# zovoilis-lab/Flye

Hardware: AMD Instinct MI355X
Metric: Gbp reads overlapped/sec (higher is better)
Workload: dtype u64

## Files before the change

### flye_amd/csrc/fg_ctx.h

```cpp
#pragma once

#include <hip/hip_runtime.h>
#include <cstdint>
#include <cstdio>
#include <cstdlib>
#include <new>
#include <cstring>
#include <string>
#include <vector>
#include <map>
#include <memory>
#include <condition_variable>
#include <functional>
#include <mutex>
#include <thread>
#include <atomic>
#include <algorithm>

#include "../../include/flye_gpu.h"
#include "fg_error.h"

typedef uint64_t u64;
typedef uint32_t u32;
typedef uint16_t u16;
// ... 255 lines not shown

	bool indexBuilt = false;
	float sampleRate = 1.0f;
	u64 nKeys = 0, nEntries = 0, nRep = 0, tableSlots = 0;
	DevBuf<u64> dKeys;
	DevBuf<u64> dKeyOff;
	DevBuf<u64> dEntries;
	DevBuf<u64> dRepKeys;
	DevBuf<u64> dTable;
	bool tableWide = false;
	FgTable table{};
	DevBuf<u32> dIndexedBits;
	DevBuf<u32> dMaybeBits;
	u32 shardWorld = 1, shardRank = 0;

	std::unique_ptr<fg_ctx> lane2;
	std::shared_ptr<void> indexBuild;
	bool gathering = false;
	DevBuf<u64> gKeys, gKeyOff, gEntries, gRepKeys;
	u64 gNKeys = 0, gNEntries = 0, gNRep = 0;
	u32 splitWorld = 0;
	DevBuf<u64> sCounts, sEntries;
	bool scattering = false;
	u32 scatterWorld = 1, scatterRank = 0;

	DevBuf<u32> dQuery;
	u64 hitCapHint = 0;
	const u32* curQuery = nullptr;
	DevBuf<u64> dQKmerOff;
	DevBuf<u64> dProbe;
	DevBuf<u64> dPartK0, dPartV0, dPartK1, dPartV1;
	DevBuf<char> dPartScratch;
	DevBuf<unsigned long long> dPartCount;
	DevBuf<u64> dHitOff;
	DevBuf<u64> dFiltOff;
	DevBuf<i32> dFiltPos;
	DevBuf<u64> dHitKey;
	DevBuf<u32> dHitVal;
	DevBuf<u16> dHitVal16;
	bool hitVal16 = false;
	DevBuf<u32> dHitKey32;
	DevBuf<i32> dScore, dBack;
	DevBuf<int4> dCand;
	DevBuf<u64> dGroupStart;
	DevBuf<u32> dGroupQuery;
	DevBuf<u32> dGroupExt, dGroupFirstCur, dGroupLastCur;
	DevBuf<uint8_t> dGroupExtSorted;
	DevBuf<u32> dTmp32;
	DevBuf<fg_seed_hit> dSeedHits;
	DevBuf<u64> dRecvRun, dRecvIdx;
	DevBuf<u32> dRecvErr;
	DevBuf<u64> dCntA, dCntB, dGroupCnt, dGroupOff, dPrimCnt, dPrimOff, dDpGroups, dDpElems;
	DevBuf<u32> dPrimFlag, dDpSize, dListSmall, dListBig, dListDp, dListFused, dListCnt;
	DevBuf<u32> dCur, dExt;
	DevBuf<char> dPrimOut;
	DevBuf<u64> dPrimNode, dPrimBase, dMatchSize, dMatchOff, dMatches;
	DevBuf<u32> dMatchCnt;
	PinnedBuf<u64> hMatches, hMatchOff;
	PinnedBuf<u32> hMatchCnt;
	DevBuf<char> dSortTasks, dSortBig;
	DevBuf<unsigned long long> dSmallElems;
	DevBuf<unsigned long long> dLazyCnt;
	DevBuf<u32> dSortCnt;
	DevBuf<u32> dTieFree;
	u32 tieFreeQ0 = 0, tieFreeN = 0;
	DevBuf<u32> dSortFree, dSortReason;
	u32 sortReasonN = 0;
	u32 sortRadixSegs = 0;
	DevBuf<int> dEditScratch;
	DevBuf<u32> dEditList;
	DevBuf<char> dEditCnt;
	DevBuf<u64> dEditSlab;
	DevBuf<char> dEditPrims;
	DevBuf<u32> dEditQuery;
	DevBuf<i32> dEditOut;
	DevBuf<char> dRangeSides;
	DevBuf<i32> dRangeLen;
	DevBuf<u64> dRangeOff;
	DevBuf<uint8_t> dRangeTrg, dRangeQry;
	DevBuf<u32> dDecCnt;
	DevBuf<u64> dDecOff;
	DevBuf<uint8_t> dDecOps;
	DevBuf<i32> dDecLens;
	DevBuf<i32> dTrimPre;
	DevBuf<u64> dTrimRowCnt, dTrimRowOff, dTrimScan, dTrimKeys, dTrimIvl, dTrimSeg, dTrimAcc, dTrimAccOff;
	DevBuf<unsigned long long> dTrimPairCnt;
	DevBuf<u32> dTrimVals, dTrimAccCnt, dTrimKept;
	DevBuf<char> dTrimRaw, dTrimOut;
	DevBuf<u32> dRcNodes, dRcVals, dRcU32;
	DevBuf<char> dRcTab, dRcAln;
	DevBuf<u64> dRcOff, dRcKeys, dRcOut;
	DevBuf<i32> dRcOutScore;
	DevBuf<char> dCovRecs, dCovSort;
	DevBuf<u64> dCovIv, dCovKeys, dCovOff;
	DevBuf<i32> dCovI32, dCovVec;
	DevBuf<char> dPolBytes, dPolCand, dPolItems, dPolTasks, dPolRes;
	DevBuf<u64> dPolOff, dPolEdOff;
	DevBuf<long long> dPolScore, dPolCells, dPolEdits;
	DevBuf<char> dBub[36];
	DevBuf<char> dCc[40];
	DevBuf<char> dCig[20];
	DevBuf<char> dDv[28];
	DevBuf<char> dPt[36];
	PinnedBuf<char> hPrim;
	PinnedBuf<u64> hOff;
	PinnedBuf<u64> hScalar;
// ... 2 lines not shown
	~fg_ctx()
	{
		if (evFork) (void)hipEventDestroy(evFork);
		if (evJoin) (void)hipEventDestroy(evJoin);
		if (evJoin3) (void)hipEventDestroy(evJoin3);
		if (evOff) (void)hipEventDestroy(evOff);
		for (auto e : evPiece) if (e) (void)hipEventDestroy(e);
		if (stream2) (void)hipStreamDestroy(stream2);
		if (stream3) (void)hipStreamDestroy(stream3);
		if (stream) (void)hipStreamDestroy(stream);
	}
};

#if defined(__HIPCC__)

__device__ __forceinline__ i32 fg_uni(i32 v) { return __builtin_amdgcn_readfirstlane(v); }
__device__ __forceinline__ u32 fg_uni(u32 v) { return (u32)__builtin_amdgcn_readfirstlane((int)v); }
__device__ __forceinline__ u64 fg_uni(u64 v)
{
	return ((u64)(u32)__builtin_amdgcn_readfirstlane((int)(u32)(v >> 32)) << 32) |
		   (u32)__builtin_amdgcn_readfirstlane((int)(u32)v);
}

#define FG_PK_VALBITS 24
struct PK {
	u64 v;
	PK() = default;
	__host__ __device__ PK(int x) : v((u64)(unsigned)x) {}
	__host__ __device__ explicit PK(u64 x) : v(x) {}
};
__device__ __forceinline__ bool operator<(const PK& a, const PK& b) { return (a.v >> FG_PK_VALBITS) < (b.v >> FG_PK_VALBITS); }
__device__ __forceinline__ bool operator>(const PK& a, const PK& b) { return (a.v >> FG_PK_VALBITS) > (b.v >> FG_PK_VALBITS); }
__device__ __forceinline__ bool operator<=(const PK& a, const PK& b) { return (a.v >> FG_PK_VALBITS) <= (b.v >> FG_PK_VALBITS); }
__device__ __forceinline__ bool operator>=(const PK& a, const PK& b) { return (a.v >> FG_PK_VALBITS) >= (b.v >> FG_PK_VALBITS); }
__device__ __forceinline__ bool operator==(const PK& a, const PK& b) { return a.v == b.v; }
__device__ __forceinline__ bool operator!=(const PK& a, const PK& b) { return a.v != b.v; }

struct NoVal {
	struct Ref {
		__device__ __forceinline__ operator u32() const { return 0u; }
		__device__ __forceinline__ const Ref& operator=(u32) const { return *this; }
	};
	__device__ __forceinline__ Ref operator[](long long) const { return Ref{}; }
	__device__ __forceinline__ NoVal operator+(long long) const { return NoVal{}; }
};

struct K32V16;
template <class KT> struct HitKeyView;
template <> struct HitKeyView<u64> {
	const u64* k; const u32* v; int curBits; u32 firstId;
	__device__ __forceinline__ u32 ext(u64 i) const { return (u32)(k[i] >> 32); }
	__device__ __forceinline__ u32 ext_raw(u64 i) const { return (u32)(k[i] >> 32); }
	__device__ __forceinline__ u32 cur(u64 i) const { return (u32)k[i]; }
	__device__ __forceinline__ u32 val(u64 i) const { return v[i]; }
};
template <> struct HitKeyView<u32> {
	const u32* k; const u32* v; int curBits; u32 firstId;
	__device__ __forceinline__ u32 ext(u64 i) const { return (k[i] >> curBits) + firstId; }
	__device__ __forceinline__ u32 ext_raw(u64 i) const { return k[i] >> curBits; }
	__device__ __forceinline__ u32 cur(u64 i) const { return k[i] & ((1u << curBits) - 1u); }
	__device__ __forceinline__ u32 val(u64 i) const { return v[i]; }
};
template <> struct HitKeyView<K32V16> {
	const u32* k; const u16* v; int curBits; u32 firstId;
	__device__ __forceinline__ u32 ext(u64 i) const { return (k[i] >> curBits) + firstId; }
	__device__ __forceinline__ u32 ext_raw(u64 i) const { return k[i] >> curBits; }
	__device__ __forceinline__ u32 cur(u64 i) const { return k[i] & ((1u << curBits) - 1u); }
	__device__ __forceinline__ u32 val(u64 i) const { return v[i]; }
};
template <> struct HitKeyView<PK> {
	const PK* k; const u32* v; int curBits; u32 firstId;
	__device__ __forceinline__ u32 ext(u64 i) const { return (u32)(k[i].v >> (FG_PK_VALBITS + curBits)) + firstId; }
	__device__ __forceinline__ u32 ext_raw(u64 i) const { return (u32)(k[i].v >> (FG_PK_VALBITS + curBits)); }
	__device__ __forceinline__ u32 cur(u64 i) const { return (u32)(k[i].v >> FG_PK_VALBITS) & ((1u << curBits) - 1u); }
	__device__ __forceinline__ u32 val(u64 i) const { return (u32)k[i].v & ((1u << FG_PK_VALBITS) - 1u); }
};

__device__ __forceinline__ u64 fg_mix(u64 x)
{
	x ^= x >> 33; x *= 0xff51afd7ed558ccdULL; x ^= x >> 33;
	x *= 0xc4ceb9fe1a85ec53ULL; x ^= x >> 33;
	return x;
}

__device__ __forceinline__ u32 fg_base_at(const u64* __restrict__ w, i32 L, bool rc, i32 pos)
{
	const i32 p = rc ? L - 1 - pos : pos;
	const u32 b = (u32)((w[p >> 5] >> ((p & 31) * 2)) & 3);
	return rc ? (~b & 3) : b;
}

__device__ __forceinline__ u64 fg_range_step(const u64* __restrict__ w, i32 L, bool rc, i32 start, i32 len, bool hpc,
											 i32 t0, u32& carry, u32& b, bool& keep)
{
	const int lane = threadIdx.x & 63;
	const i32 t = t0 + lane;
	const bool valid = t < len;
	b = valid ? fg_base_at(w, L, rc, start + t) : 0u;
	u32 prev = __shfl_up(b, 1);
	if (lane == 0) prev = carry;
	keep = valid && (!hpc || prev != b);
	carry = __shfl(b, 63);
	return __builtin_amdgcn_ballot_w64(keep);
}

__device__ __forceinline__ u64 fg_kmer_hash(u64 x)
{
	u64 z = (x += 0x9E3779B97F4A7C15ULL);
	z = (z ^ (z >> 30)) * 0xBF58476D1CE4E5B9ULL;
	z = (z ^ (z >> 27)) * 0x94D049BB133111EBULL;
	return z ^ (z >> 31);
}

__device__ __forceinline__ u64 fg_chunk(const u64* __restrict__ w, i32 q, int k)
{
	const int sh = (q & 31) * 2;
	u64 lo = w[q >> 5] >> sh;
	if (sh + 2 * k > 64) lo |= w[(q >> 5) + 1] << (64 - sh);
	return (k == 32) ? lo : (lo & ((1ULL << (2 * k)) - 1));
}

__device__ __forceinline__ u64 fg_rev2(u64 x, int k)
{
	u64 r = __brevll(x);
	r = ((r >> 1) & 0x5555555555555555ULL) | ((r & 0x5555555555555555ULL) << 1);
	return r >> (64 - 2 * k);
}
// ... 192 lines not shown
```

### flye_amd/csrc/fg_overlap.hip

```cpp
#include "fg_ctx.h"
#include "fg_wavesort.h"
#include "fg_devprim.h"
#include "fg_taskchain.h"
#include <atomic>

#include <algorithm>
#include <cmath>
#include <chrono>
#include <functional>
#include <thread>
#include <type_traits>

#define WG 256
#define FLAG_SELF (1ULL << 63)
#define FLAG_FLIP (1ULL << 62)
#define OFF_MASK ((1ULL << 38) - 1)

namespace {

__device__ __forceinline__ u32 block_exscan(u32 v, u32* sh , u32* total)
{
	const int lane = threadIdx.x & 63, w = threadIdx.x >> 6;
	u32 inc = v;
	for (int o = 1; o < 64; o <<= 1)
// ... 1031 lines not shown
	}
}

__global__ void k_prim_gather(const u64* __restrict__ groupOff, const u32* __restrict__ primCount,
							  const u64* __restrict__ groupStart, const u32* __restrict__ groupExt,
							  const u32* __restrict__ gCur, const u32* __restrict__ gExt, const int4* __restrict__ cand,
							  const i32* __restrict__ len, u32 firstId, int k,
							  const u64* __restrict__ filtOff, const i32* __restrict__ filtPos,
							  const u64* __restrict__ primOff, PrimRec* __restrict__ out,
							  u64* __restrict__ primNode, u64* __restrict__ primBase, u64* __restrict__ matchSize)
{
	__shared__ u32 sh[WG / 64 + 1];
	const u32 q = blockIdx.x;
	const u64 b = groupOff[q], e = groupOff[q + 1];
	u64 obase = primOff[q];
	const i32* fp = filtPos + filtOff[q];
	const i32 nf = (i32)(filtOff[q + 1] - filtOff[q]);
	for (u64 i0 = b; i0 < e; i0 += WG)
	{
		const u64 g = i0 + threadIdx.x;
		const u32 cnt = g < e ? primCount[g] : 0u;
		u32 tot;
		const u32 pos = block_exscan(cnt, sh, &tot);
		if (cnt)
		{
			const u64 g0 = groupStart[g];
			const u32 extId = groupExt[g];
			const i32 extLen = len[(extId - firstId) >> 1];
			for (u32 a = 0; a < cnt; ++a)
			{
				const int4 c4 = cand[g0 + a];
				PrimRec r;
				r.query = q; r.extId = extId;
				r.curBegin = (i32)gCur[g0 + c4.x]; r.extBegin = (i32)gExt[g0 + c4.x];
				r.curEnd = (i32)gCur[g0 + c4.y] + k - 1; r.extEnd = (i32)gExt[g0 + c4.y] + k - 1;
				r.extLen = extLen; r.score = c4.w; r.chainLength = c4.z;
				i32 lo = 0, hi = nf;
				while (lo < hi) { const i32 m = (lo + hi) >> 1; if (fp[m] < r.curBegin) lo = m + 1; else hi = m; }
				const i32 first = lo;
				hi = nf;
				while (lo < hi) { const i32 m = (lo + hi) >> 1; if (fp[m] <= r.curEnd) lo = m + 1; else hi = m; }
				r.filtered = lo - first;
				r.editDistance = -1; r.hpcLenCur = 0; r.hpcLenExt = 0;
				out[obase + pos + a] = r;
				if (primNode)
				{
					primNode[obase + pos + a] = g0 + (u64)c4.y;
					primBase[obase + pos + a] = g0;
					matchSize[obase + pos + a] = (u64)c4.z + 2;
				}
			}
		}
		obase += tot;
	}
}

__global__ void k_chain_matches(const PrimRec* __restrict__ prims, u64 nPrim, const u64* __restrict__ primNode,
								const u64* __restrict__ primBase, const u64* __restrict__ matchOff,
								const u32* __restrict__ gCur, const u32* __restrict__ gExt,
								const i32* __restrict__ gBack, int k, u64* __restrict__ matches,
								u32* __restrict__ matchCnt)
{
	const u64 p = (u64)blockIdx.x * blockDim.x + threadIdx.x;
	if (p >= nPrim) return;
	const PrimRec r = prims[p];
	const u64 base = primBase[p];
	u64* slot = matches + matchOff[p];
	const i32 ub = r.chainLength + 2;
	i32 pos = (i32)(primNode[p] - base);
	i32 kept = 0, lastCur = 0;
	for (i32 step = 0; step < r.chainLength; ++step)
	{
		const i32 cu = (i32)gCur[base + pos];
		if (kept == 0 || lastCur - cu > k)
		{
			slot[ub - 2 - kept] = (u64)(u32)cu | ((u64)gExt[base + pos] << 32);
			lastCur = cu;
			++kept;
		}
		pos = gBack[base + pos];
	}
	slot[ub - 2 - kept] = (u64)(u32)r.curBegin | ((u64)(u32)r.extBegin << 32);
	slot[ub - 1] = (u64)(u32)r.curEnd | ((u64)(u32)r.extEnd << 32);
	matchCnt[p] = (u32)kept + 2;
}

template <class T>
T fetchScalar(fg_ctx* c, const T* dptr)
{
	static_assert(sizeof(T) <= 8, "scalar");
	c->hScalar.reserve(8);
	HIP_CHECK(hipMemcpyAsync(c->hScalar.p, dptr, sizeof(T), hipMemcpyDeviceToHost, c->stream));
	HIP_CHECK(hipStreamSynchronize(c->stream));
	T v;
	memcpy(&v, c->hScalar.p, sizeof(T));
	return v;
}

}

struct SortRadixStats { u64 segments, hits; };

#define SORT_MAX_LEVELS 128
template <class KT>
static bool sortRadixUsable(int recBits)
{
// ... 459 lines not shown
	while ((1ULL << recBits) < 2ULL * c->nReads) ++recBits;
	const bool key32 = curBits + recBits <= 32 && !getenv("FG_FORCE_KEY64");
	c->tieFreeN = 0; c->sortReasonN = 0;
	const bool canPack = recBits + curBits + FG_PK_VALBITS <= 64 && c->maxLen < (1 << FG_PK_VALBITS);
	const bool wantPack = !(getenv("FG_PACKED_KEYS") && atoi(getenv("FG_PACKED_KEYS")) == 0);
	const int keyMode = key32 ? 0 : ((canPack && wantPack) ? 1 : 2);
	const bool val16 = keyMode == 0 && !recv && c->maxLen <= 65536 && !(getenv("FG_VAL16") && atoi(getenv("FG_VAL16")) == 0);
	c->hitVal16 = val16;
	if (keyMode == 0)
	{
		c->dHitKey32.reserve(hitCap + 1); c->dTieFree.reserve(nq + 1);
		if (val16) c->dHitVal16.reserve(hitCap + 2); else c->dHitVal.reserve(hitCap + 1);
		if (recv) recvFill<u32>(c, recv, callQ0, sub0, nq, nHits, curBits, c->dHitKey32.p, c->dHitVal.p);
		else { ScopedK t(c->timer, "k_fill");
		  if (val16)
			  hipLaunchKernelGGL((k_fill<u32, u16>), nq, WG, 0, s, dQuery, c->dLen.p, qLen, dQKmerOff, k, c->firstId, curBits,
								 c->dProbe.p, c->dEntries.p, c->dHitOff.p, c->dFiltOff.p, c->dHitKey32.p, c->dHitVal16.p, c->dFiltPos.p, c->dTieFree.p);
		  else
			  hipLaunchKernelGGL(k_fill<u32>, nq, WG, 0, s, dQuery, c->dLen.p, qLen, dQKmerOff, k, c->firstId, curBits,
								 c->dProbe.p, c->dEntries.p, c->dHitOff.p, c->dFiltOff.p, c->dHitKey32.p, c->dHitVal.p, c->dFiltPos.p, c->dTieFree.p); }
		if (!recv) { c->tieFreeQ0 = callQ0 + sub0; c->tieFreeN = nq; }
		const u32* sortFree = recv ? nullptr : c->dTieFree.p;
		if (sortFree && nHits)
		{
			c->dSortFree.reserve(nq + 1); c->dSortReason.reserve(nq + 1);
			if (sortScreen(c, c->dHitOff.p, nq, c->dHitKey32.p, curBits, recBits, c->dTieFree.p, fgChainMinUnique(p), p->min_overlap,
						   c->dSortFree.p, c->dSortReason.p))
				{ sortFree = c->dSortFree.p; c->sortReasonN = nq; }
		}
		if (val16) sortSegments<u32, u16>(c, c->dHitOff.p, nq, c->dHitKey32.p, c->dHitVal16.p, nHits, curBits, sortFree, recBits);
		else sortSegments<u32>(c, c->dHitOff.p, nq, c->dHitKey32.p, c->dHitVal.p, nHits, curBits, sortFree, recBits);
	}
	else if (keyMode == 1)
	{
		c->dHitKey.reserve(hitCap + 1);
		if (recv) recvFill<PK>(c, recv, callQ0, sub0, nq, nHits, curBits, (PK*)c->dHitKey.p, (u32*)nullptr);
		else { ScopedK t(c->timer, "k_fill");
		  hipLaunchKernelGGL(k_fill<PK>, nq, WG, 0, s, dQuery, c->dLen.p, qLen, dQKmerOff, k, c->firstId, curBits,
							 c->dProbe.p, c->dEntries.p, c->dHitOff.p, c->dFiltOff.p, (PK*)c->dHitKey.p, (u32*)nullptr, c->dFiltPos.p, (u32*)nullptr); }
		sortSegments<PK>(c, c->dHitOff.p, nq, (PK*)c->dHitKey.p, (u32*)nullptr, nHits, curBits);
	}
	else
	{
		c->dHitKey.reserve(hitCap + 1); c->dHitVal.reserve(hitCap + 1);
		if (recv) recvFill<u64>(c, recv, callQ0, sub0, nq, nHits, curBits, c->dHitKey.p, c->dHitVal.p);
		else { ScopedK t(c->timer, "k_fill");
		  hipLaunchKernelGGL(k_fill<u64>, nq, WG, 0, s, dQuery, c->dLen.p, qLen, dQKmerOff, k, c->firstId, 0,
							 c->dProbe.p, c->dEntries.p, c->dHitOff.p, c->dFiltOff.p, c->dHitKey.p, c->dHitVal.p, c->dFiltPos.p, (u32*)nullptr); }
		sortSegments<u64>(c, c->dHitOff.p, nq, c->dHitKey.p, c->dHitVal.p, nHits, curBits);
	}
	const HitKeyView<u32> hk32{c->dHitKey32.p, c->dHitVal.p, curBits, c->firstId};
	const HitKeyView<u64> hk64{c->dHitKey.p, c->dHitVal.p, curBits, c->firstId};
	const HitKeyView<PK> hkp{(const PK*)c->dHitKey.p, nullptr, curBits, c->firstId};
	{ ScopedK t(c->timer, "k_group_count");
	  if (keyMode == 0) hipLaunchKernelGGL(k_group_count<u32>, nq, WG, 0, s, c->dHitOff.p, hk32, c->dGroupCnt.p);
	  else if (keyMode == 1) hipLaunchKernelGGL(k_group_count<PK>, nq, WG, 0, s, c->dHitOff.p, hkp, c->dGroupCnt.p);
	  else hipLaunchKernelGGL(k_group_count<u64>, nq, WG, 0, s, c->dHitOff.p, hk64, c->dGroupCnt.p); }
	{ ScopedK t(c->timer, "k_exscan");
	  hipLaunchKernelGGL(k_exscan, 1, 1024, 0, s, c->dGroupCnt.p, c->dGroupOff.p, nq); }
	const u64 nGroups = fetchScalar(c, c->dGroupOff.p + nq);
	if (nGroups >= 0xFFFFFFFFULL) throw FgError{FG_ERR_ARG, "too many target groups in one chunk"};
	c->dGroupStart.reserve(nGroups + 1); c->dGroupQuery.reserve(nGroups + 1);
	c->dGroupExt.reserve(nGroups + 1); c->dGroupFirstCur.reserve(nGroups + 1); c->dGroupLastCur.reserve(nGroups + 1);
	c->dPrimFlag.reserve(nGroups + 1); c->dDpSize.reserve(nGroups + 1);
	{ ScopedK t(c->timer, "k_group_fill");
	  if (keyMode == 0) hipLaunchKernelGGL(k_group_fill<u32>, nq, WG, 0, s, c->dHitOff.p, hk32, c->dGroupOff.p, c->dGroupStart.p,
										   c->dGroupQuery.p, c->dGroupExt.p, c->dGroupFirstCur.p, c->dGroupLastCur.p);
	  else if (keyMode == 1) hipLaunchKernelGGL(k_group_fill<PK>, nq, WG, 0, s, c->dHitOff.p, hkp, c->dGroupOff.p, c->dGroupStart.p,
												c->dGroupQuery.p, c->dGroupExt.p, c->dGroupFirstCur.p, c->dGroupLastCur.p);
	  else hipLaunchKernelGGL(k_group_fill<u64>, nq, WG, 0, s, c->dHitOff.p, hk64, c->dGroupOff.p, c->dGroupStart.p,
							  c->dGroupQuery.p, c->dGroupExt.p, c->dGroupFirstCur.p, c->dGroupLastCur.p); }
	fgChainStage(c, p, forceLocal, nGroups, nHits, keyMode, curBits);
	c->dSmallElems.reserve(1);
	HIP_CHECK(hipMemsetAsync(c->dSmallElems.p, 0, 8, s));
	{ ScopedK t(c->timer, "k_prim_count");
	  hipLaunchKernelGGL(k_prim_count, nq, WG, 0, s, c->dGroupOff.p, c->dPrimFlag.p, c->dDpSize.p, c->dPrimCnt.p,
						 c->dDpGroups.p, c->dDpElems.p, c->dGroupStart.p, nGroups, nHits, fgChainSmallMax(), c->dSmallElems.p); }
	{ ScopedK t(c->timer, "k_exscan");
	  hipLaunchKernelGGL(k_exscan, 1, 1024, 0, s, c->dPrimCnt.p, c->dPrimOff.p, nq); }
	const u64 nPrim = fetchScalar(c, c->dPrimOff.p + nq);
	c->dPrimOut.reserve((nPrim + 1) * sizeof(PrimRec));
	const bool keepAln = p->keep_alignment;
	if (keepAln) { c->dPrimNode.reserve(nPrim + 1); c->dPrimBase.reserve(nPrim + 1); c->dMatchSize.reserve(nPrim + 1);
				   c->dMatchOff.reserve(nPrim + 2); c->dMatchCnt.reserve(nPrim + 1); }
	{ ScopedK t(c->timer, "k_prim_gather");
	  hipLaunchKernelGGL(k_prim_gather, nq, WG, 0, s, c->dGroupOff.p, c->dPrimFlag.p, c->dGroupStart.p, c->dGroupExt.p,
						 c->dCur.p, c->dExt.p, c->dCand.p, c->dLen.p, c->firstId, k, c->dFiltOff.p, c->dFiltPos.p,
						 c->dPrimOff.p, (PrimRec*)c->dPrimOut.p, keepAln ? c->dPrimNode.p : (u64*)nullptr,
						 keepAln ? c->dPrimBase.p : (u64*)nullptr, keepAln ? c->dMatchSize.p : (u64*)nullptr); }
	if (p->nucl_alignment) fgEditDistances(c, (PrimRec*)c->dPrimOut.p, nPrim, p->use_hpc);
	res->nMatchSlots = 0;
	if (keepAln && nPrim)
	{
		if (nPrim >= 0xFFFFFFFFULL) throw FgError{FG_ERR_ARG, "too many overlaps in one chunk"};
		{ ScopedK t(c->timer, "k_exscan");
		  hipLaunchKernelGGL(k_exscan, 1, 1024, 0, s, c->dMatchSize.p, c->dMatchOff.p, (u32)nPrim); }
		const u64 slots = fetchScalar(c, c->dMatchOff.p + nPrim);
		res->nMatchSlots = slots;
		c->dMatches.reserve(slots + 1);
		{ ScopedK t(c->timer, "k_chain_matches");
		  hipLaunchKernelGGL(k_chain_matches, (unsigned)((nPrim + WG - 1) / WG), WG, 0, s, (const PrimRec*)c->dPrimOut.p, nPrim,
							 c->dPrimNode.p, c->dPrimBase.p, c->dMatchOff.p, c->dCur.p, c->dExt.p, c->dBack.p, k,
							 c->dMatches.p, c->dMatchCnt.p); }
		c->hMatches.reserve(slots + 1); c->hMatchOff.reserve(nPrim + 1); c->hMatchCnt.reserve(nPrim + 1);
		ScopedK t(c->timer, "copy_results_d2h");
		HIP_CHECK(hipMemcpyAsync(c->hMatches.p, c->dMatches.p, slots * 8, hipMemcpyDeviceToHost, s));
		HIP_CHECK(hipMemcpyAsync(c->hMatchOff.p, c->dMatchOff.p, (nPrim + 1) * 8, hipMemcpyDeviceToHost, s));
		HIP_CHECK(hipMemcpyAsync(c->hMatchCnt.p, c->dMatchCnt.p, nPrim * 4, hipMemcpyDeviceToHost, s));
	}
	if ((primBase + nPrim + 1) * sizeof(PrimRec) > c->hPrim.n)
	{
		HIP_CHECK(hipStreamSynchronize(s));
		c->hPrim.reserveKeep((primBase + nPrim + 1) * sizeof(PrimRec), primBase * sizeof(PrimRec));
	}
	c->hOff.reserve(3 * (size_t)(nq + 1) + 1);
	{ ScopedK t(c->timer, "copy_results_d2h");
	  HIP_CHECK(hipMemcpyAsync(c->hOff.p, c->dPrimOff.p, (nq + 1) * 8ULL, hipMemcpyDeviceToHost, s));
	  HIP_CHECK(hipMemcpyAsync(c->hOff.p + (nq + 1), c->dDpGroups.p, nq * 8ULL, hipMemcpyDeviceToHost, s));
	  HIP_CHECK(hipMemcpyAsync(c->hOff.p + 2 * (size_t)(nq + 1), c->dDpElems.p, nq * 8ULL, hipMemcpyDeviceToHost, s));
	  HIP_CHECK(hipMemcpyAsync(c->hOff.p + 3 * (size_t)(nq + 1), c->dSmallElems.p, 8, hipMemcpyDeviceToHost, s));
	  HIP_CHECK(hipEventRecord(c->evOff, s));
	  static const int wantPieces = getenv("FG_D2H_PIECES") ? std::max(1, std::min(FG_D2H_MAX_PIECES, atoi(getenv("FG_D2H_PIECES")))) : 12;
	  const int nPieces = nPrim >= 100000 ? wantPieces : 1;
	  for (int i = 0; i < nPieces; ++i)
	  {
		  const u64 a = nPrim * i / nPieces, b = nPrim * (i + 1) / nPieces;
		  if (b > a)
			  HIP_CHECK(hipMemcpyAsync(c->hPrim.p + (primBase + a) * sizeof(PrimRec), c->dPrimOut.p + a * sizeof(PrimRec),
									   (b - a) * sizeof(PrimRec), hipMemcpyDeviceToHost, s));
		  HIP_CHECK(hipEventRecord(c->evPiece[i], s));
		  c->pieceEnd[i] = primBase + b;
	  }
	  c->nPieces = nPieces; }
	HIP_CHECK(hipEventSynchronize(c->evOff));
	if (keepAln) HIP_CHECK(hipStreamSynchronize(s));
	res->nPrim = nPrim;
	res->dpGroups = 0; res->dpElems = 0;
	res->dpElemsSmall = c->hOff.p[3 * (size_t)(nq + 1)];
	for (u32 i = 0; i < nq; ++i) { res->dpGroups += c->hOff.p[(nq + 1) + i]; res->dpElems += c->hOff.p[2 * (size_t)(nq + 1) + i]; }
}

static void stageBudgets(fg_ctx* c, u64& kmerBudget, u64& hitBudget)
{
	kmerBudget = getenv("FG_KMER_BUDGET") ? strtoull(getenv("FG_KMER_BUDGET"), nullptr, 10) : (1ULL << 30);
	hitBudget = getenv("FG_HIT_BUDGET") ? strtoull(getenv("FG_HIT_BUDGET"), nullptr, 10) : (3ULL << 29);
	if (!getenv("FG_KMER_BUDGET") && !getenv("FG_HIT_BUDGET"))
	{
		size_t freeB = 0, totalB = 0;
		HIP_CHECK(hipMemGetInfo(&freeB, &totalB));
		const u64 held = c->dHitKey.bytes() + c->dHitKey32.bytes() + c->dHitVal.bytes() + c->dHitVal16.bytes() + c->dCur.bytes() + c->dExt.bytes() +
						 c->dScore.bytes() + c->dBack.bytes() + c->dTmp32.bytes() + c->dCand.bytes() + c->dProbe.bytes();
		const u64 avail = (u64)freeB + held;
		const u64 usable = avail > (8ULL << 30) ? (avail - (4ULL << 30)) / 10 * 9 : avail / 2;
		hitBudget = std::min(hitBudget, std::max<u64>(16ULL << 20, usable / 100 * 85 / 80));
		kmerBudget = std::min(kmerBudget, std::max<u64>(16ULL << 20, usable / 100 * 15 / 9));
	}
}

static fg_ctx* laneTwo(fg_ctx* c)
{
	if (!c->lane2)
	{
		std::unique_ptr<fg_ctx> l(new fg_ctx);
		l->device = c->device;
		if (hipStreamCreateWithFlags(&l->stream, hipStreamNonBlocking) != hipSuccess ||
			hipStreamCreateWithFlags(&l->stream2, hipStreamNonBlocking) != hipSuccess ||
			hipStreamCreateWithFlags(&l->stream3, hipStreamNonBlocking) != hipSuccess ||
			hipEventCreateWithFlags(&l->evJoin3, hipEventDisableTiming) != hipSuccess ||
			hipEventCreateWithFlags(&l->evOff, hipEventDisableTiming) != hipSuccess ||
			hipEventCreateWithFlags(&l->evFork, hipEventDisableTiming) != hipSuccess ||
			hipEventCreateWithFlags(&l->evJoin, hipEventDisableTiming) != hipSuccess)
			throw FgError{FG_ERR_HIP, "streams of the second lane"};
		for (auto& e : l->evPiece)
			if (hipEventCreateWithFlags(&e, hipEventDisableTiming) != hipSuccess) throw FgError{FG_ERR_HIP, "events of the second lane"};
		l->timer.stream = l->stream;
		c->lane2 = std::move(l);
	}
	fg_ctx* l = c->lane2.get();
	l->k = c->k; l->nReads = c->nReads; l->firstId = c->firstId; l->maxLen = c->maxLen;
	l->totalKmers = c->totalKmers; l->totalBases = c->totalBases;
	l->hasQ = c->hasQ; l->nQReads = c->nQReads; l->qFirstId = c->qFirstId; l->qMaxLen = c->qMaxLen;
	l->indexBuilt = c->indexBuilt; l->sampleRate = c->sampleRate; l->nKeys = c->nKeys; l->nEntries = c->nEntries; l->nRep = c->nRep;
	l->tableSlots = c->tableSlots; l->tableWide = c->tableWide; l->table = c->table;
	l->timer.enabled = c->timer.enabled;
	l->dWords.alias(c->dWords); l->dWordOff.alias(c->dWordOff); l->dLen.alias(c->dLen); l->dKmerOff.alias(c->dKmerOff);
	l->dQWords.alias(c->dQWords); l->dQWordOff.alias(c->dQWordOff); l->dQLen.alias(c->dQLen);
	l->dKeyOff.alias(c->dKeyOff); l->dEntries.alias(c->dEntries); l->dTable.alias(c->dTable); l->dIndexedBits.alias(c->dIndexedBits); l->dMaybeBits.alias(c->dMaybeBits);
	l->dQuery.alias(c->dQuery); l->dQKmerOff.alias(c->dQKmerOff); l->dProbe.alias(c->dProbe);
	l->dCntA.alias(c->dCntA); l->dCntB.alias(c->dCntB);
	l->dLazyCnt.alias(c->dLazyCnt);
	return l;
}
// ... 475 lines not shown
```

Before: 5.406.

## Flatten group count/fill and primitive scan over hits instead of per-query blocks

Replaces the per-query block launches for group counting, group filling, primitive counting and gathering with flat tile-parallel kernels over all hits, each thread handling 8 consecutive keys. Query boundaries inside a tile are found by binary search and marked in shared memory. The single-block exscan is replaced by a device-wide scan, and per-group primitive positions come from scanning the primitive flags. DP totals are now reduced on the device with atomics instead of being summed on the host from per-query arrays. This removes load imbalance from skewed query sizes and the serial single-block scan, at the cost of extra kernels such as the groupOff binary search and more code paths.

```diff
diff --git a/flye_amd/csrc/fg_ctx.h b/flye_amd/csrc/fg_ctx.h
--- a/flye_amd/csrc/fg_ctx.h
+++ b/flye_amd/csrc/fg_ctx.h
@@ -331,6 +331,7 @@
 	DevBuf<u32> dRecvErr;
 	DevBuf<u64> dCntA, dCntB, dGroupCnt, dGroupOff, dPrimCnt, dPrimOff, dDpGroups, dDpElems;
 	DevBuf<u32> dPrimFlag, dDpSize, dListSmall, dListBig, dListDp, dListFused, dListCnt;
+	DevBuf<u32> dTileCnt, dPrimPos, dScanScratch;
 	DevBuf<u32> dCur, dExt;
 	DevBuf<char> dPrimOut;
 	DevBuf<u64> dPrimNode, dPrimBase, dMatchSize, dMatchOff, dMatches;
@@ -439,6 +440,11 @@
 	__device__ __forceinline__ u32 ext(u64 i) const { return (u32)(k[i] >> 32); }
 	__device__ __forceinline__ u32 ext_raw(u64 i) const { return (u32)(k[i] >> 32); }
 	__device__ __forceinline__ u32 cur(u64 i) const { return (u32)k[i]; }
+	typedef u64 Word;
+	__device__ __forceinline__ u64 key(u64 i) const { return k[i]; }
+	__device__ __forceinline__ u32 ext_of(u64 x) const { return (u32)(x >> 32); }
+	__device__ __forceinline__ u32 ext_raw_of(u64 x) const { return (u32)(x >> 32); }
+	__device__ __forceinline__ u32 cur_of(u64 x) const { return (u32)x; }
 	__device__ __forceinline__ u32 val(u64 i) const { return v[i]; }
 };
 template <> struct HitKeyView<u32> {
@@ -446,6 +452,11 @@
 	__device__ __forceinline__ u32 ext(u64 i) const { return (k[i] >> curBits) + firstId; }
 	__device__ __forceinline__ u32 ext_raw(u64 i) const { return k[i] >> curBits; }
 	__device__ __forceinline__ u32 cur(u64 i) const { return k[i] & ((1u << curBits) - 1u); }
+	typedef u32 Word;
+	__device__ __forceinline__ u32 key(u64 i) const { return k[i]; }
+	__device__ __forceinline__ u32 ext_of(u32 x) const { return (x >> curBits) + firstId; }
+	__device__ __forceinline__ u32 ext_raw_of(u32 x) const { return x >> curBits; }
+	__device__ __forceinline__ u32 cur_of(u32 x) const { return x & ((1u << curBits) - 1u); }
 	__device__ __forceinline__ u32 val(u64 i) const { return v[i]; }
 };
 template <> struct HitKeyView<K32V16> {
@@ -453,6 +464,11 @@
 	__device__ __forceinline__ u32 ext(u64 i) const { return (k[i] >> curBits) + firstId; }
 	__device__ __forceinline__ u32 ext_raw(u64 i) const { return k[i] >> curBits; }
 	__device__ __forceinline__ u32 cur(u64 i) const { return k[i] & ((1u << curBits) - 1u); }
+	typedef u32 Word;
+	__device__ __forceinline__ u32 key(u64 i) const { return k[i]; }
+	__device__ __forceinline__ u32 ext_of(u32 x) const { return (x >> curBits) + firstId; }
+	__device__ __forceinline__ u32 ext_raw_of(u32 x) const { return x >> curBits; }
+	__device__ __forceinline__ u32 cur_of(u32 x) const { return x & ((1u << curBits) - 1u); }
 	__device__ __forceinline__ u32 val(u64 i) const { return v[i]; }
 };
 template <> struct HitKeyView<PK> {
@@ -460,6 +476,11 @@
 	__device__ __forceinline__ u32 ext(u64 i) const { return (u32)(k[i].v >> (FG_PK_VALBITS + curBits)) + firstId; }
 	__device__ __forceinline__ u32 ext_raw(u64 i) const { return (u32)(k[i].v >> (FG_PK_VALBITS + curBits)); }
 	__device__ __forceinline__ u32 cur(u64 i) const { return (u32)(k[i].v >> FG_PK_VALBITS) & ((1u << curBits) - 1u); }
+	typedef u64 Word;
+	__device__ __forceinline__ u64 key(u64 i) const { return k[i].v; }
+	__device__ __forceinline__ u32 ext_of(u64 x) const { return (u32)(x >> (FG_PK_VALBITS + curBits)) + firstId; }
+	__device__ __forceinline__ u32 ext_raw_of(u64 x) const { return (u32)(x >> (FG_PK_VALBITS + curBits)); }
+	__device__ __forceinline__ u32 cur_of(u64 x) const { return (u32)(x >> FG_PK_VALBITS) & ((1u << curBits) - 1u); }
 	__device__ __forceinline__ u32 val(u64 i) const { return (u32)k[i].v & ((1u << FG_PK_VALBITS) - 1u); }
 };
 
diff --git a/flye_amd/csrc/fg_overlap.hip b/flye_amd/csrc/fg_overlap.hip
--- a/flye_amd/csrc/fg_overlap.hip
+++ b/flye_amd/csrc/fg_overlap.hip
@@ -1107,6 +1107,227 @@
 			}
 		}
 		obase += tot;
+	}
+}
+
+constexpr int FG_GROUP_GF = 8;
+constexpr int FG_GROUP_TILE = WG * FG_GROUP_GF;
+constexpr u32 NO_QUERY = 0xFFFFFFFFu;
+
+template <int GF>
+__device__ __forceinline__ u32 tile_query_starts(const u64* __restrict__ hitOff, u32 nq, u64 tileBegin, u64 tileEnd,
+												 u32* shStartQ )
+{
+#pragma unroll
+	for (int t = 0; t < GF; ++t) shStartQ[t * WG + threadIdx.x] = NO_QUERY;
+	u32 lo = 0, hi = nq;
+	while (hi - lo > 1)
+	{
+		const u32 m = lo + ((hi - lo) >> 1);
+		if (fg_uni(hitOff[m]) <= tileBegin) lo = m; else hi = m;
+	}
+	const u32 q0 = lo;
+	__syncthreads();
+	if (threadIdx.x == 0 && hitOff[q0] == tileBegin) shStartQ[0] = q0;
+	for (u32 q = q0 + 1 + threadIdx.x; q < nq; q += WG)
+	{
+		const u64 b = hitOff[q];
+		if (b >= tileEnd) break;
+		if (hitOff[q + 1] > b) shStartQ[(u32)(b - tileBegin)] = q;
+	}
+	__syncthreads();
+	return q0;
+}
+
+template <class KT> using HitKeyWord = typename HitKeyView<KT>::Word;
+template <class KT, int GF>
+__device__ __forceinline__ u32 tile_heads(const u64* __restrict__ hitOff, u32 nq, const HitKeyView<KT>& hitKey, u64 nHits,
+										  u32* shStartQ, u64& first, u64& tileEnd, HitKeyWord<KT> (&key)[GF + 1], bool (&head)[GF],
+										  u32 (&mark)[GF])
+{
+	const u64 tileBegin = (u64)blockIdx.x * (WG * GF);
+	tileEnd = tileBegin + WG * GF < nHits ? tileBegin + WG * GF : nHits;
+	first = tileBegin + (u64)threadIdx.x * GF;
+	const u64 last = tileEnd - 1;
+	const u64 prev = first ? first - 1 : 0;
+	key[0] = hitKey.key(prev < last ? prev : last);
+	if (tileEnd - tileBegin == WG * GF)
+	{
+#pragma unroll
+		for (int t = 0; t < GF; ++t) key[t + 1] = hitKey.key(first + t);
+	}
+	else
+	{
+#pragma unroll
+		for (int t = 0; t < GF; ++t) key[t + 1] = hitKey.key(first + t < last ? first + t : last);
+	}
+	const u32 q0 = tile_query_starts<GF>(hitOff, nq, tileBegin, tileEnd, shStartQ);
+#pragma unroll
+	for (int t = 0; t < GF; ++t)
+	{
+		mark[t] = shStartQ[threadIdx.x * GF + t];
+		head[t] = first + t < tileEnd &&
+				  (mark[t] != NO_QUERY || hitKey.ext_raw_of(key[t + 1]) != hitKey.ext_raw_of(key[t]));
+	}
+	return q0;
+}
+
+template <class KT, int GF>
+__global__ void __launch_bounds__(WG) k_group_count_flat(const u64* __restrict__ hitOff, u32 nq, HitKeyView<KT> hitKey, u64 nHits,
+														 u32* __restrict__ tileCnt)
+{
+	__shared__ u32 shStartQ[WG * GF];
+	__shared__ u32 sh[WG / 64];
+	u64 first, tileEnd;
+	HitKeyWord<KT> key[GF + 1];
+	bool head[GF];
+	u32 mark[GF];
+	(void)tile_heads<KT, GF>(hitOff, nq, hitKey, nHits, shStartQ, first, tileEnd, key, head, mark);
+	u32 c = 0;
+#pragma unroll
+	for (int t = 0; t < GF; ++t) c += head[t];
+	for (int o = 32; o > 0; o >>= 1) c += __shfl_down(c, o);
+	if ((threadIdx.x & 63) == 0) sh[threadIdx.x >> 6] = c;
+	__syncthreads();
+	if (threadIdx.x == 0)
+	{
+		u32 t = 0;
+		for (int i = 0; i < WG / 64; ++i) t += sh[i];
+		tileCnt[blockIdx.x] = t;
+		if (blockIdx.x == 0) tileCnt[gridDim.x] = 0;
+	}
+}
+
+template <class KT, int GF>
+__global__ void __launch_bounds__(WG) k_group_fill_flat(const u64* __restrict__ hitOff, u32 nq, HitKeyView<KT> hitKey, u64 nHits,
+														const u32* __restrict__ tileBase, u64 nGroups, u64* __restrict__ groupStart,
+														u32* __restrict__ groupQuery, u32* __restrict__ groupExt,
+														u32* __restrict__ groupFirstCur, u32* __restrict__ groupLastCur)
+{
+	__shared__ u32 shStartQ[WG * GF];
+	__shared__ u32 shS[WG / 64], shM[WG / 64];
+	u64 first, tileEnd;
+	HitKeyWord<KT> key[GF + 1];
+	bool head[GF];
+	u32 mark[GF];
+	const u32 base = tileBase[blockIdx.x];
+	const u32 q0 = tile_heads<KT, GF>(hitOff, nq, hitKey, nHits, shStartQ, first, tileEnd, key, head, mark);
+	u32 nHead = 0, lastQ = 0;
+#pragma unroll
+	for (int t = 0; t < GF; ++t) { nHead += head[t]; if (mark[t] != NO_QUERY) lastQ = mark[t] + 1; }
+	const int lane = threadIdx.x & 63, w = threadIdx.x >> 6;
+	u32 incS = nHead, incM = lastQ;
+#pragma unroll
+	for (int o = 1; o < 64; o <<= 1)
+	{
+		const u32 tS = __shfl_up(incS, o), tM = __shfl_up(incM, o);
+		if (lane >= o) { incS += tS; incM = tM > incM ? tM : incM; }
+	}
+	if (lane == 63) { shS[w] = incS; shM[w] = incM; }
+	u32 curQ = __shfl_up(incM, 1);
+	if (lane == 0) curQ = 0;
+	__syncthreads();
+	u32 pos = incS - nHead;
+	for (int i = 0; i < w; ++i) { pos += shS[i]; curQ = shM[i] > curQ ? shM[i] : curQ; }
+	u64 g = (u64)base + pos;
+#pragma unroll
+	for (int t = 0; t < GF; ++t)
+	{
+		const u64 i = first + t;
+		if (mark[t] != NO_QUERY) curQ = mark[t] + 1;
+		if (head[t])
+		{
+			groupStart[g] = i; groupQuery[g] = curQ ? curQ - 1 : q0;
+			groupExt[g] = hitKey.ext_of(key[t + 1]); groupFirstCur[g] = hitKey.cur_of(key[t + 1]);
+			if (i > 0) groupLastCur[g - 1] = hitKey.cur_of(key[t]);
+			++g;
+		}
+		if (i + 1 == nHits) groupLastCur[nGroups - 1] = hitKey.cur_of(key[t + 1]);
+	}
+}
+
+__global__ void k_group_off(const u64* __restrict__ hitOff, u32 nq, const u64* __restrict__ groupStart, u64 nGroups,
+							u64* __restrict__ groupOff)
+{
+	const u32 q = blockIdx.x * blockDim.x + threadIdx.x;
+	if (q > nq) return;
+	const u64 h = hitOff[q];
+	u64 lo = 0, hi = nGroups;
+	while (lo < hi) { const u64 m = (lo + hi) >> 1; if (groupStart[m] < h) lo = m + 1; else hi = m; }
+	groupOff[q] = lo;
+}
+
+constexpr unsigned PRIM_COUNT_BLOCKS = 1024;
+__global__ void __launch_bounds__(WG) k_prim_count_flat(const u32* __restrict__ dpSize, const u64* __restrict__ groupStart,
+														u64 nGroups, u64 nHits, u32 smallMax, unsigned long long* __restrict__ totals,
+														const u64* __restrict__ groupOff, const u32* __restrict__ primPos, u32 nq,
+														u64* __restrict__ primOff)
+{
+	__shared__ u64 sh[3][WG / 64];
+	const u64 stride = (u64)gridDim.x * WG;
+	for (u64 q = (u64)blockIdx.x * WG + threadIdx.x; q <= nq; q += stride) primOff[q] = primPos[groupOff[q]];
+	u64 dg = 0, de = 0, ds = 0;
+	for (u64 g = (u64)blockIdx.x * WG + threadIdx.x; g < nGroups; g += stride)
+	{
+		const u32 d = dpSize[g];
+		dg += d != 0; de += d;
+		if (d && smallMax)
+		{
+			const u64 n = (g + 1 < nGroups ? groupStart[g + 1] : nHits) - groupStart[g];
+			ds += n <= smallMax ? d : 0u;
+		}
+	}
+	for (int o = 32; o > 0; o >>= 1) { dg += __shfl_down(dg, o); de += __shfl_down(de, o); ds += __shfl_down(ds, o); }
+	if ((threadIdx.x & 63) == 0) { sh[0][threadIdx.x >> 6] = ds; sh[1][threadIdx.x >> 6] = dg; sh[2][threadIdx.x >> 6] = de; }
+	__syncthreads();
+	if (threadIdx.x < 3)
+	{
+		u64 t = 0;
+		for (int i = 0; i < WG / 64; ++i) t += sh[threadIdx.x][i];
+		if (t) atomicAdd(totals + threadIdx.x, (unsigned long long)t);
+	}
+}
+
+__global__ void k_prim_gather_flat(u64 nGroups, const u32* __restrict__ primCount, const u32* __restrict__ primPos,
+								   const u32* __restrict__ groupQuery, const u64* __restrict__ groupStart,
+								   const u32* __restrict__ groupExt, const u32* __restrict__ gCur, const u32* __restrict__ gExt,
+								   const int4* __restrict__ cand, const i32* __restrict__ len, u32 firstId, int k,
+								   const u64* __restrict__ filtOff, const i32* __restrict__ filtPos, PrimRec* __restrict__ out,
+								   u64* __restrict__ primNode, u64* __restrict__ primBase, u64* __restrict__ matchSize)
+{
+	const u64 g = (u64)blockIdx.x * blockDim.x + threadIdx.x;
+	if (g >= nGroups) return;
+	const u32 cnt = primCount[g];
+	if (!cnt) return;
+	const u32 q = groupQuery[g];
+	const u64 obase = primPos[g];
+	const i32* fp = filtPos + filtOff[q];
+	const i32 nf = (i32)(filtOff[q + 1] - filtOff[q]);
+	const u64 g0 = groupStart[g];
+	const u32 extId = groupExt[g];
+	const i32 extLen = len[(extId - firstId) >> 1];
+	for (u32 a = 0; a < cnt; ++a)
+	{
+		const int4 c4 = cand[g0 + a];
+		PrimRec r;
+		r.query = q; r.extId = extId;
+		r.curBegin = (i32)gCur[g0 + c4.x]; r.extBegin = (i32)gExt[g0 + c4.x];
+		r.curEnd = (i32)gCur[g0 + c4.y] + k - 1; r.extEnd = (i32)gExt[g0 + c4.y] + k - 1;
+		r.extLen = extLen; r.score = c4.w; r.chainLength = c4.z;
+		i32 lo = 0, hi = nf;
+		while (lo < hi) { const i32 m = (lo + hi) >> 1; if (fp[m] < r.curBegin) lo = m + 1; else hi = m; }
+		const i32 firstF = lo;
+		hi = nf;
+		while (lo < hi) { const i32 m = (lo + hi) >> 1; if (fp[m] <= r.curEnd) lo = m + 1; else hi = m; }
+		r.filtered = lo - firstF;
+		r.editDistance = -1; r.hpcLenCur = 0; r.hpcLenExt = 0;
+		out[obase + a] = r;
+		if (primNode)
+		{
+			primNode[obase + a] = g0 + (u64)c4.y;
+			primBase[obase + a] = g0;
+			matchSize[obase + a] = (u64)c4.z + 2;
+		}
 	}
 }
 
@@ -1672,17 +1893,48 @@
 	const HitKeyView<u32> hk32{c->dHitKey32.p, c->dHitVal.p, curBits, c->firstId};
 	const HitKeyView<u64> hk64{c->dHitKey.p, c->dHitVal.p, curBits, c->firstId};
 	const HitKeyView<PK> hkp{(const PK*)c->dHitKey.p, nullptr, curBits, c->firstId};
-	{ ScopedK t(c->timer, "k_group_count");
-	  if (keyMode == 0) hipLaunchKernelGGL(k_group_count<u32>, nq, WG, 0, s, c->dHitOff.p, hk32, c->dGroupCnt.p);
-	  else if (keyMode == 1) hipLaunchKernelGGL(k_group_count<PK>, nq, WG, 0, s, c->dHitOff.p, hkp, c->dGroupCnt.p);
-	  else hipLaunchKernelGGL(k_group_count<u64>, nq, WG, 0, s, c->dHitOff.p, hk64, c->dGroupCnt.p); }
-	{ ScopedK t(c->timer, "k_exscan");
-	  hipLaunchKernelGGL(k_exscan, 1, 1024, 0, s, c->dGroupCnt.p, c->dGroupOff.p, nq); }
-	const u64 nGroups = fetchScalar(c, c->dGroupOff.p + nq);
+	const bool flat = nHits < 0xFFFFFFFFULL && !(getenv("FG_GROUP_FLAT") && atoi(getenv("FG_GROUP_FLAT")) == 0);
+	const u64 nTiles = (nHits + FG_GROUP_TILE - 1) / FG_GROUP_TILE;
+	u64 nGroups = 0;
+	if (!flat)
+	{
+		{ ScopedK t(c->timer, "k_group_count");
+		  if (keyMode == 0) hipLaunchKernelGGL(k_group_count<u32>, nq, WG, 0, s, c->dHitOff.p, hk32, c->dGroupCnt.p);
+		  else if (keyMode == 1) hipLaunchKernelGGL(k_group_count<PK>, nq, WG, 0, s, c->dHitOff.p, hkp, c->dGroupCnt.p);
+		  else hipLaunchKernelGGL(k_group_count<u64>, nq, WG, 0, s, c->dHitOff.p, hk64, c->dGroupCnt.p); }
+		{ ScopedK t(c->timer, "k_exscan");
+		  hipLaunchKernelGGL(k_exscan, 1, 1024, 0, s, c->dGroupCnt.p, c->dGroupOff.p, nq); }
+		nGroups = fetchScalar(c, c->dGroupOff.p + nq);
+	}
+	else if (nTiles)
+	{
+		c->dTileCnt.reserve(nTiles + 1); c->dScanScratch.reserve(fgprim::scanScratchElems(nTiles + 1));
+		{ ScopedK t(c->timer, "k_group_count");
+		  if (keyMode == 0) hipLaunchKernelGGL((k_group_count_flat<u32, FG_GROUP_GF>), (unsigned)nTiles, WG, 0, s, c->dHitOff.p, nq, hk32, nHits, c->dTileCnt.p);
+		  else if (keyMode == 1) hipLaunchKernelGGL((k_group_count_flat<PK, FG_GROUP_GF>), (unsigned)nTiles, WG, 0, s, c->dHitOff.p, nq, hkp, nHits, c->dTileCnt.p);
+		  else hipLaunchKernelGGL((k_group_count_flat<u64, FG_GROUP_GF>), (unsigned)nTiles, WG, 0, s, c->dHitOff.p, nq, hk64, nHits, c->dTileCnt.p); }
+		{ ScopedK t(c->timer, "k_group_scan");
+		  fgprim::scan<u32>(s, c->dTileCnt.p, c->dTileCnt.p, nTiles + 1, false, c->dScanScratch.p); }
+		nGroups = fetchScalar(c, c->dTileCnt.p + nTiles);
+	}
 	if (nGroups >= 0xFFFFFFFFULL) throw FgError{FG_ERR_ARG, "too many target groups in one chunk"};
 	c->dGroupStart.reserve(nGroups + 1); c->dGroupQuery.reserve(nGroups + 1);
 	c->dGroupExt.reserve(nGroups + 1); c->dGroupFirstCur.reserve(nGroups + 1); c->dGroupLastCur.reserve(nGroups + 1);
 	c->dPrimFlag.reserve(nGroups + 1); c->dDpSize.reserve(nGroups + 1);
+	if (flat)
+	{
+		if (nTiles)
+		{ ScopedK t(c->timer, "k_group_fill");
+		  if (keyMode == 0) hipLaunchKernelGGL((k_group_fill_flat<u32, FG_GROUP_GF>), (unsigned)nTiles, WG, 0, s, c->dHitOff.p, nq, hk32, nHits, c->dTileCnt.p,
+											   nGroups, c->dGroupStart.p, c->dGroupQuery.p, c->dGroupExt.p, c->dGroupFirstCur.p, c->dGroupLastCur.p);
+		  else if (keyMode == 1) hipLaunchKernelGGL((k_group_fill_flat<PK, FG_GROUP_GF>), (unsigned)nTiles, WG, 0, s, c->dHitOff.p, nq, hkp, nHits, c->dTileCnt.p,
+													nGroups, c->dGroupStart.p, c->dGroupQuery.p, c->dGroupExt.p, c->dGroupFirstCur.p, c->dGroupLastCur.p);
+		  else hipLaunchKernelGGL((k_group_fill_flat<u64, FG_GROUP_GF>), (unsigned)nTiles, WG, 0, s, c->dHitOff.p, nq, hk64, nHits, c->dTileCnt.p,
+								  nGroups, c->dGroupStart.p, c->dGroupQuery.p, c->dGroupExt.p, c->dGroupFirstCur.p, c->dGroupLastCur.p); }
+		ScopedK t(c->timer, "k_group_off");
+		hipLaunchKernelGGL(k_group_off, (nq + 1 + WG - 1) / WG, WG, 0, s, c->dHitOff.p, nq, c->dGroupStart.p, nGroups, c->dGroupOff.p);
+	}
+	else
 	{ ScopedK t(c->timer, "k_group_fill");
 	  if (keyMode == 0) hipLaunchKernelGGL(k_group_fill<u32>, nq, WG, 0, s, c->dHitOff.p, hk32, c->dGroupOff.p, c->dGroupStart.p,
 										   c->dGroupQuery.p, c->dGroupExt.p, c->dGroupFirstCur.p, c->dGroupLastCur.p);
@@ -1691,18 +1943,50 @@
 	  else hipLaunchKernelGGL(k_group_fill<u64>, nq, WG, 0, s, c->dHitOff.p, hk64, c->dGroupOff.p, c->dGroupStart.p,
 							  c->dGroupQuery.p, c->dGroupExt.p, c->dGroupFirstCur.p, c->dGroupLastCur.p); }
 	fgChainStage(c, p, forceLocal, nGroups, nHits, keyMode, curBits);
-	c->dSmallElems.reserve(1);
-	HIP_CHECK(hipMemsetAsync(c->dSmallElems.p, 0, 8, s));
-	{ ScopedK t(c->timer, "k_prim_count");
-	  hipLaunchKernelGGL(k_prim_count, nq, WG, 0, s, c->dGroupOff.p, c->dPrimFlag.p, c->dDpSize.p, c->dPrimCnt.p,
-						 c->dDpGroups.p, c->dDpElems.p, c->dGroupStart.p, nGroups, nHits, fgChainSmallMax(), c->dSmallElems.p); }
-	{ ScopedK t(c->timer, "k_exscan");
-	  hipLaunchKernelGGL(k_exscan, 1, 1024, 0, s, c->dPrimCnt.p, c->dPrimOff.p, nq); }
-	const u64 nPrim = fetchScalar(c, c->dPrimOff.p + nq);
+	c->dSmallElems.reserve(3);
+	HIP_CHECK(hipMemsetAsync(c->dSmallElems.p, 0, 24, s));
+	u64 nPrim = 0;
+	if (flat)
+	{
+		c->dPrimPos.reserve(nGroups + 1); c->dScanScratch.reserve(fgprim::scanScratchElems(nGroups + 1));
+		HIP_CHECK(hipMemsetAsync(c->dPrimFlag.p + nGroups, 0, 4, s));
+		{ ScopedK t(c->timer, "k_prim_scan");
+		  fgprim::scan<u32>(s, c->dPrimFlag.p, c->dPrimPos.p, nGroups + 1, false, c->dScanScratch.p); }
+		c->hScalar.reserve(8);
+		HIP_CHECK(hipMemcpyAsync(c->hScalar.p, c->dPrimPos.p + nGroups, 4, hipMemcpyDeviceToHost, s));
+		HIP_CHECK(hipEventRecord(c->evOff, s));
+		{ ScopedK t(c->timer, "k_prim_count");
+		  const u64 n = std::max<u64>(nGroups, (u64)nq + 1);
+		  hipLaunchKernelGGL(k_prim_count_flat, (unsigned)std::min<u64>(PRIM_COUNT_BLOCKS, (n + WG - 1) / WG), WG, 0, s, c->dDpSize.p, c->dGroupStart.p, nGroups, nHits,
+							 fgChainSmallMax(), c->dSmallElems.p, c->dGroupOff.p, c->dPrimPos.p, nq, c->dPrimOff.p); }
+		HIP_CHECK(hipEventSynchronize(c->evOff));
+		u32 v;
+		memcpy(&v, c->hScalar.p, 4);
+		nPrim = v;
+	}
+	else
+	{
+		{ ScopedK t(c->timer, "k_prim_count");
+		  hipLaunchKernelGGL(k_prim_count, nq, WG, 0, s, c->dGroupOff.p, c->dPrimFlag.p, c->dDpSize.p, c->dPrimCnt.p,
+							 c->dDpGroups.p, c->dDpElems.p, c->dGroupStart.p, nGroups, nHits, fgChainSmallMax(), c->dSmallElems.p); }
+		{ ScopedK t(c->timer, "k_exscan");
+		  hipLaunchKernelGGL(k_exscan, 1, 1024, 0, s, c->dPrimCnt.p, c->dPrimOff.p, nq); }
+		nPrim = fetchScalar(c, c->dPrimOff.p + nq);
+	}
 	c->dPrimOut.reserve((nPrim + 1) * sizeof(PrimRec));
 	const bool keepAln = p->keep_alignment;
 	if (keepAln) { c->dPrimNode.reserve(nPrim + 1); c->dPrimBase.reserve(nPrim + 1); c->dMatchSize.reserve(nPrim + 1);
 				   c->dMatchOff.reserve(nPrim + 2); c->dMatchCnt.reserve(nPrim + 1); }
+	if (flat)
+	{
+		if (nPrim)
+		{ ScopedK t(c->timer, "k_prim_gather");
+		  hipLaunchKernelGGL(k_prim_gather_flat, (unsigned)((nGroups + WG - 1) / WG), WG, 0, s, nGroups, c->dPrimFlag.p, c->dPrimPos.p,
+							 c->dGroupQuery.p, c->dGroupStart.p, c->dGroupExt.p, c->dCur.p, c->dExt.p, c->dCand.p, c->dLen.p, c->firstId, k,
+							 c->dFiltOff.p, c->dFiltPos.p, (PrimRec*)c->dPrimOut.p, keepAln ? c->dPrimNode.p : (u64*)nullptr,
+							 keepAln ? c->dPrimBase.p : (u64*)nullptr, keepAln ? c->dMatchSize.p : (u64*)nullptr); }
+	}
+	else
 	{ ScopedK t(c->timer, "k_prim_gather");
 	  hipLaunchKernelGGL(k_prim_gather, nq, WG, 0, s, c->dGroupOff.p, c->dPrimFlag.p, c->dGroupStart.p, c->dGroupExt.p,
 						 c->dCur.p, c->dExt.p, c->dCand.p, c->dLen.p, c->firstId, k, c->dFiltOff.p, c->dFiltPos.p,
@@ -1733,12 +2017,15 @@
 		HIP_CHECK(hipStreamSynchronize(s));
 		c->hPrim.reserveKeep((primBase + nPrim + 1) * sizeof(PrimRec), primBase * sizeof(PrimRec));
 	}
-	c->hOff.reserve(3 * (size_t)(nq + 1) + 1);
+	c->hOff.reserve(3 * (size_t)(nq + 1) + 3);
 	{ ScopedK t(c->timer, "copy_results_d2h");
 	  HIP_CHECK(hipMemcpyAsync(c->hOff.p, c->dPrimOff.p, (nq + 1) * 8ULL, hipMemcpyDeviceToHost, s));
-	  HIP_CHECK(hipMemcpyAsync(c->hOff.p + (nq + 1), c->dDpGroups.p, nq * 8ULL, hipMemcpyDeviceToHost, s));
-	  HIP_CHECK(hipMemcpyAsync(c->hOff.p + 2 * (size_t)(nq + 1), c->dDpElems.p, nq * 8ULL, hipMemcpyDeviceToHost, s));
-	  HIP_CHECK(hipMemcpyAsync(c->hOff.p + 3 * (size_t)(nq + 1), c->dSmallElems.p, 8, hipMemcpyDeviceToHost, s));
+	  if (!flat)
+	  {
+		  HIP_CHECK(hipMemcpyAsync(c->hOff.p + (nq + 1), c->dDpGroups.p, nq * 8ULL, hipMemcpyDeviceToHost, s));
+		  HIP_CHECK(hipMemcpyAsync(c->hOff.p + 2 * (size_t)(nq + 1), c->dDpElems.p, nq * 8ULL, hipMemcpyDeviceToHost, s));
+	  }
+	  HIP_CHECK(hipMemcpyAsync(c->hOff.p + 3 * (size_t)(nq + 1), c->dSmallElems.p, 24, hipMemcpyDeviceToHost, s));
 	  HIP_CHECK(hipEventRecord(c->evOff, s));
 	  static const int wantPieces = getenv("FG_D2H_PIECES") ? std::max(1, std::min(FG_D2H_MAX_PIECES, atoi(getenv("FG_D2H_PIECES")))) : 12;
 	  const int nPieces = nPrim >= 100000 ? wantPieces : 1;
@@ -1757,7 +2044,8 @@
 	res->nPrim = nPrim;
 	res->dpGroups = 0; res->dpElems = 0;
 	res->dpElemsSmall = c->hOff.p[3 * (size_t)(nq + 1)];
-	for (u32 i = 0; i < nq; ++i) { res->dpGroups += c->hOff.p[(nq + 1) + i]; res->dpElems += c->hOff.p[2 * (size_t)(nq + 1) + i]; }
+	if (flat) { res->dpGroups = c->hOff.p[3 * (size_t)(nq + 1) + 1]; res->dpElems = c->hOff.p[3 * (size_t)(nq + 1) + 2]; }
+	else for (u32 i = 0; i < nq; ++i) { res->dpGroups += c->hOff.p[(nq + 1) + i]; res->dpElems += c->hOff.p[2 * (size_t)(nq + 1) + i]; }
 }
 
 static void stageBudgets(fg_ctx* c, u64& kmerBudget, u64& hitBudget)
```

Result: faster. 5.550, median of 6 (+2.7%).
